# wushan270/mit-6.824-2015

Measured on AMD Instinct MI355X. Metric: word-count input GB/s (whole node) and % of HBM roofline at 1/2/4/8 MI355X, higher is better.
Workload: dtype u8

## Files before the change

__graft_entry__.py:

```python
from __future__ import annotations

import os
import shutil
import subprocess
import sys

ROOT = os.path.dirname(os.path.abspath(__file__))
PKG = os.path.join(ROOT, "mit-6.824-2015_amd")
CSRC = os.path.join(PKG, "csrc")
OUT = os.path.join(PKG, "wcg")
ORACLE = os.path.join(ROOT, "oracle")

HIPCC = os.environ.get("HIPCC", "/opt/rocm/bin/hipcc" if os.path.exists("/opt/rocm/bin/hipcc") else "hipcc")
HIP_FLAGS = ["--offload-arch=gfx950", "-O3", "-std=c++17", "-shared", "-fPIC", "-fvisibility=hidden", "-pthread"]
HIP_LIBS = ["-L/opt/rocm/lib", "-lrccl"]


def _run(cmd):
    print("+", " ".join(cmd), flush=True)
    subprocess.run(cmd, check=True)


def _stale(target, sources):
    if not os.path.exists(target):
# ... 4 lines not shown

def _sources(d, exts):
    return [os.path.join(d, f) for f in sorted(os.listdir(d)) if f.endswith(exts)]


def _check_isa() -> None:
    import tempfile
    sys.path.insert(0, os.path.join(ROOT, "tools"))
    import check_inflight
    with tempfile.TemporaryDirectory() as td:
        s = os.path.join(td, "wcg.s")
        _run([HIPCC, "--offload-arch=gfx950", "-O3", "-std=c++17", "--cuda-device-only", "-S", "-o", s,
              os.path.join(CSRC, "wcg_api.hip")])
        text = open(s).read()
    errors = []
    for sym in ("_ZN3wcg5k_mapILi0ELb1EEEvNS_7MapArgsE", "_ZN3wcg5k_mapILi0ELb0EEEvNS_7MapArgsE", "_ZN3wcg5k_aggILi0EEEvNS_7AggArgsENS_7MapArgsE",
                "_ZN3wcg5k_aggILi1EEEvNS_7AggArgsENS_7MapArgsE"):
        errors += check_inflight.check(text, sym)[0]
    if errors:
        lib = os.path.join(OUT, "libwcg.so")
        os.remove(lib)
        raise RuntimeError("k_map prefetch register discipline broken:\n" + "\n".join(errors))


def build(force: bool = False) -> None:
    hip_deps = _sources(CSRC, (".hip", ".h")) + [os.path.join(ROOT, "include", "wcg.h")]
    lib = os.path.join(OUT, "libwcg.so")
    if force or _stale(lib, hip_deps):
        _run([HIPCC, *HIP_FLAGS, "-o", lib, os.path.join(CSRC, "wcg_api.hip"), *HIP_LIBS])
        _check_isa()
    gen = os.path.join(OUT, "libgencorpus.so")
    gsrc = os.path.join(CSRC, "gencorpus.c")
# ... 45 lines not shown
```

include/wcg.h:

```cpp
#ifndef WCG_H
#define WCG_H

#include <stdint.h>

#ifdef __cplusplus
extern "C" {
#endif

#ifndef WCG_API
#define WCG_API __attribute__((visibility("default")))
#endif

typedef struct wcg_ctx wcg_ctx;

enum {
    WCG_OK = 0,
    WCG_EINVAL = 1,
    WCG_ENOMEM = 2,
    WCG_EHIP = 3,
    WCG_EFULL = 4,
    WCG_ESTATE = 5
};

enum {
// ... 81 lines not shown

WCG_API int wcg_index_merged(wcg_ctx *ctx, uint64_t *nlines);

WCG_API int wcg_load_merged(wcg_ctx *ctx, const uint8_t *host_bytes, uint64_t n, uint64_t *nlines);
WCG_API int wcg_load_merged_device(wcg_ctx *ctx, const void *dev_bytes, uint64_t n, uint64_t *nlines);

WCG_API int wcg_timings(wcg_ctx *ctx, double *ms, int n, uint64_t *map_launches);
WCG_API int wcg_enable_timing(wcg_ctx *ctx, int on);

WCG_API int wcg_stats(wcg_ctx *ctx, uint64_t *stats9);

WCG_API int wcg_ingest_stats(wcg_ctx *ctx, double *out, int n);

WCG_API int wcg_reduce_path(const wcg_ctx *ctx, int *path);

WCG_API uint32_t wcg_ihash(const uint8_t *key, uint64_t len);

WCG_API const char *wcg_version(void);

#ifdef __cplusplus
}
#endif
#endif
```

mit-6.824-2015_amd/csrc/wcg_api.hip:

```cpp
#include <hip/hip_ext.h>
#include <hip/hip_runtime.h>
#include <rccl/rccl.h>

#include <fcntl.h>
#include <sys/stat.h>
#include <unistd.h>

#include <algorithm>
#include <array>
#include <chrono>
#include <cstdio>
#include <cstdlib>
#include <cstring>
#include <memory>
#include <string>
#include <thread>
#include <tuple>
#include <vector>

#include "../../include/wcg.h"
#include "wcg_common.h"
#include "wcg_map.h"
#include "wcg_agg.h"
#include "wcg_reduce.h"
#include "wcg_top.h"
#include "wcg_query.h"
#include "wcg_index.h"
#include "wcg_fused.h"
#include "wcg_ingest.h"

using namespace wcg;

struct wcg_ctx {
    int device = 0;
    int ncu = 256;
    hipStream_t own_stream = nullptr;
    hipStream_t stream = nullptr;
    hipStream_t long_stream = nullptr;
    hipEvent_t ev_fork = nullptr, ev_join = nullptr;
    u64 max_input = 0, max_keys = 0;
    GEntry* gtab = nullptr; u64 gslots = 0;
    GEntry* ltab = nullptr; u64 lslots = 0;
    uint8_t* arena = nullptr; u64 arena_cap = 0;
// ... 102 lines not shown
    hipEvent_t phase_ev[6] = {};
    u64 map_launches_since_reset = 0;
    int timing_mode = 0;
    std::vector<std::array<hipEvent_t, 5>> phase_jobs;
    bool phase_rec = false;
    std::vector<std::tuple<int, hipEvent_t, hipEvent_t>> xev;
    double acc[10] = {};
    u64 map_launches = 0;
    uint8_t* fr_buf = nullptr;
    FrArgs fr{};
    u32 fr_epoch = 0;
    bool fused_last = false;
    bool pending = false;
    uint16_t* flist = nullptr; u64 flist_cap = 0;
    u64* h_st_dev = nullptr;
    std::string err;
};

namespace {

#define HIPCHK(ctx, call)                                                                   \
    do {                                                                                    \
        hipError_t e_ = (call);                                                             \
        if (e_ != hipSuccess) {                                                             \
            (ctx)->err = std::string(#call) + ": " + hipGetErrorString(e_);                 \
            return WCG_EHIP;                                                                \
        }                                                                                   \
    } while (0)

#define RC(call)                                                                            \
// ... 162 lines not shown
        k_compact<<<(unsigned)cdiv(std::max<u64>(total, 1), CP_NT * CP_IPT), CP_NT, 0, c->stream>>>(
            c->gtab, gs, c->ltab, ls, c->arena, c->recA, c->rec_cap, c->st, nullptr, glist, llist);
        HIPCHK(c, hipGetLastError());
        if (c->timing_all) { c->phase_ev[1] = take_event(c); HIPCHK(c, hipEventRecord(c->phase_ev[1], c->stream)); }
        RC(check_status(c));
        c->nrec = c->h_st->nrec;
        if (c->nrec <= c->rec_cap) break;
        RC(ensure_recs(c, c->nrec));
    }
    c->crec = c->recA;
    c->compacted = true;
    return WCG_OK;
}

u64 merged_bound(wcg_ctx* c, u64 n, bool json);

bool fused_eligible(wcg_ctx* c) {
    static const char* env = getenv("WCG_FUSED");
    static const bool exact_env = getenv("WCG_EXACT_REDUCE") != nullptr || getenv("WCG_SORT_TARGET") != nullptr;
    if (env && atoi(env) == 0) return false;
    return !c->compacted && !c->two_pass_used && !exact_env && c->nrec_hint >= 2 &&
           c->nrec_hint <= FR_NMAX;
}

int reduce_fused(wcg_ctx* c) {
    const u64 total = c->gslots + c->lslots;
    RC(ensure_recs(c, total));
    c->dev_sized = true;
    RC(ensure(c, &c->d_out, &c->out_cap, merged_bound(c, total, false) + 64));
    if (!c->fr_buf) {
// ... 15 lines not shown
    }
    if (!c->counts_clean) HIPCHK(c, hipMemsetAsync(&c->st->nrec, 0, 2 * sizeof(u64), c->stream));
    c->counts_clean = false;
    FrArgs a = c->fr;
    a.gtab = c->gtab; a.gslots = c->gslots; a.ltab = c->ltab; a.lslots = c->lslots;
    a.arena = c->arena; a.st = c->st; a.total_out = c->d_scalar;
    a.rec = c->recA; a.rec_cap = c->rec_cap; a.out_rec = c->recB; a.out = c->d_out;
    c->fr_epoch = (c->fr_epoch + 1) & 0xFFFFFF;
    if (c->fr_epoch == 0) c->fr_epoch = 1;
    a.epoch = c->fr_epoch;
    const char* tenv = getenv("WCG_FUSED_TARGET");
    a.target = tenv ? (u32)std::max(1, atoi(tenv)) : FR_TARGET;
    a.nitems0 = (u32)cdiv(total, (u64)CP_NT * CP_IPT);
    if (c->timing_all) { c->phase_ev[2] = take_event(c); HIPCHK(c, hipEventRecord(c->phase_ev[2], c->stream)); }
    static const bool fclock = getenv("WCG_FUSED_CLOCK") != nullptr;
    static u64* d_fclk = nullptr;
    const unsigned fgrid = (unsigned)(2 * c->ncu);
    a.clk = nullptr;
    if (fclock) {
        if (!d_fclk) HIPCHK(c, hipMalloc(&d_fclk, ((u64)fgrid * FR_CLK + 8ull * FR_NPH * FR_CLK_ITEMS + 8ull * FR_NPH) * sizeof(u64)));
        HIPCHK(c, hipMemsetAsync(d_fclk, 0, ((u64)fgrid * FR_CLK + 8ull * FR_NPH * FR_CLK_ITEMS + 8ull * FR_NPH) * sizeof(u64), c->stream));
        a.clk = d_fclk;
    }
    if (!c->h_st_dev) HIPCHK(c, hipHostGetDevicePointer((void**)&c->h_st_dev, c->h_st, 0));
    a.host_st = c->h_st_dev;
    k_fused_reduce<<<fgrid, FR_NT, 0, c->stream>>>(a);
    HIPCHK(c, hipGetLastError());
    if (fclock) {
        std::vector<u64> h((u64)fgrid * FR_CLK + 8ull * FR_NPH * FR_CLK_ITEMS + 8ull * FR_NPH);
        HIPCHK(c, hipMemcpyAsync(h.data(), d_fclk, h.size() * sizeof(u64), hipMemcpyDeviceToHost, c->stream));
        HIPCHK(c, hipStreamSynchronize(c->stream));
        u64 t0 = ~0ull, tend = 0;
        for (unsigned w = 0; w < fgrid; w++) { t0 = std::min(t0, h[w * FR_CLK]); }
        fprintf(stderr, "wcg fused clock (us from the first workgroup's start):");
        for (int p = 0; p < FR_NPH; p++) {
// ... 65 lines not shown
                std::vector<double> v = d[k];
                std::sort(v.begin(), v.end());
                fprintf(stderr, "%s %.1f/%.1f/%.1f  ", nm[k], v[v.size() / 2], v[v.size() * 9 / 10], v.back());
            }
            fprintf(stderr, "\n");
            if (!slow.empty()) {
                std::sort(slow.begin(), slow.end());
                fprintf(stderr, "  P%d slowest items (us, records):", p);
                for (size_t k = slow.size() > 6 ? slow.size() - 6 : 0; k < slow.size(); k++)
                    fprintf(stderr, " %.1f/%llu", slow[k].first, (unsigned long long)slow[k].second);
                fprintf(stderr, "; median item %.1f/%llu\n", slow[slow.size() / 2].first, (unsigned long long)slow[slow.size() / 2].second);
            }
        }
    }
    if (c->timing_all) { c->phase_ev[3] = take_event(c); HIPCHK(c, hipEventRecord(c->phase_ev[3], c->stream)); }
    c->dev_sized = false;
    c->compacted = false;
    c->fused_last = true;
    return WCG_OK;
}

int reduce_fused_finish(wcg_ctx* c) {
    HIPCHK(c, hipStreamSynchronize(c->stream));
    c->sorted = c->recB;
    c->crec = c->recA;
    c->nrec = c->nkeys = c->h_st->nrec;
    c->out_len = *c->h_scalar;
    if (c->h_st->bad_input || c->h_st->overflow || c->h_st->spin_fail) {
        c->nrec = 0; c->out_len = 0; c->reduced = false;
        RC(check_status(c));
    }
    c->nrec_hint = c->nrec;
    c->long_hint = c->h_st->long_tokens;
    c->sorted_live = true;
    c->sorted_n = c->nrec;
    return WCG_OK;
}

int resolve(wcg_ctx* c) {
    if (!c->pending) return WCG_OK;
    c->pending = false;
    return reduce_fused_finish(c);
}

int dbg(wcg_ctx* c, const char* what) {
    static const bool on = getenv("WCG_DEBUG") != nullptr;
    if (!on) return WCG_OK;
    HIPCHK(c, hipStreamSynchronize(c->stream));
    fprintf(stderr, "wcg: %s done\n", what);
    return WCG_OK;
}
// ... 469 lines not shown
    if (c->ev_fork) (void)hipEventDestroy(c->ev_fork);
    if (c->ev_join) (void)hipEventDestroy(c->ev_join);
    for (auto e : c->ev_pool) (void)hipEventDestroy(e);
    for (int i = 0; i < INGEST_SLOTS; i++) {
        if (c->ev_copied[i]) (void)hipEventDestroy(c->ev_copied[i]);
    for (auto e : c->ing_ev) (void)hipEventDestroy(e);
        if (c->ev_mapped[i]) (void)hipEventDestroy(c->ev_mapped[i]);
        if (c->hb[i]) (void)hipHostFree(c->hb[i]);
        if (c->db[i]) (void)hipFree(c->db[i]);
    }
    void* bufs[] = {c->gtab, c->ltab, c->arena, c->st, c->recA, c->recB, c->lens, c->d_out,
                    c->d_part, c->owner, c->d_per_rank, c->exp_buf, c->pool, c->region_len, c->wg_stats,
                    c->llog, c->llog_len, c->smp, c->bid, c->spx, c->irec, c->lent, c->lpcur, c->spill, c->spill_len, c->pool2, c->rlen2, c->remit, c->ovf, c->hist, c->spart, c->ikey, c->iidx, c->groups,
                    c->pid, c->d_partb, c->nlpos, c->d_rb, c->d_b0, c->d_jin, c->d_jout, c->jhist, c->dbig,
                    c->d_xrow, c->xrecv, c->grecv, c->glist, c->llist, c->fr_buf, c->flist,
                    c->top_cand, c->top_rec, c->d_top, c->q_keys, c->q_off, c->q_cnt, c->rs_part, c->d_range};
    if (c->comm) (void)ncclCommDestroy(c->comm);
    for (void* b : bufs) if (b) (void)hipFree(b);
    if (c->h_x) (void)hipHostFree(c->h_x);
    if (c->h_st) (void)hipHostFree(c->h_st);
    if (c->h_cur) (void)hipHostFree(c->h_cur);
    if (c->h_rb) (void)hipHostFree(c->h_rb);
    if (c->copy_stream) (void)hipStreamDestroy(c->copy_stream);
    if (c->own_stream) (void)hipStreamDestroy(c->own_stream);
    if (c->long_stream) (void)hipStreamDestroy(c->long_stream);
    delete c;
    return WCG_OK;
}

int wcg_set_stream(wcg_ctx* c, void* stream) {
    if (!c) return WCG_EINVAL;
// ... 161 lines not shown
            fprintf(stderr, "wcg k_agg clock: %s workgroups %u, dur mean %.1f max %.1f us, units mean %.0f\n",
                    kind ? "medium" : "short", kn[kind], kd[kind] / kn[kind] / 100.0, km[kind] / 100.0, ku[kind] / kn[kind]);
    fprintf(stderr, "wcg k_agg clock: span %.1f us, wg dur mean %.1f max %.1f us (bi %u: %llu units, start +%.1f us), "
            "units mean %.0f max %.0f\n", (t1 - t0) / 100.0, sd / nb1 / 100.0, md / 100.0, bmax,
            (unsigned long long)units[bmax], (clk[2 * bmax] - t0) / 100.0, su / nb1, mu);
    return WCG_OK;
}

}

extern "C" {

int wcg_reset(wcg_ctx* c) {
    if (!c) return WCG_EINVAL;
    c->pending = false;
    int rc = set_dev(c);
    if (rc) return rc;
    if (c->timing_mode >= 2 && c->ev_used >= EV_FOLD) {
        HIPCHK(c, hipStreamSynchronize(c->stream));
        sum_events(c, c->acc);
        c->map_ev.clear(); c->agg_ev.clear(); c->phase_jobs.clear(); c->xev.clear();
        c->ev_used = 0;
    }
    RC(reset_tables(c));
    if (c->timing_mode < 2) {
        c->map_ev.clear();
        c->agg_ev.clear();
        c->xev.clear();
        c->ev_used = 0;
        c->phase_rec = false;
// ... 79 lines not shown
        c->llog_len = nullptr; c->llog_len_cap = 0;
        HIPCHK(c, hipMalloc(&c->llog_len, grid * sizeof(u32)));
        c->llog_len_cap = grid;
    }
    a.llog = c->llog;
    a.llog_len = c->llog_len;
    const bool two_pass = two_pass0;
    const u64 rec_cap_emit = emit_log_cap(c);
    RC(ensure(c, &c->remit, &c->remit_cap, emit_log_alloc(c)));
    a.emit = two_pass ? c->remit : nullptr;
    a.emit_cap = rec_cap_emit;
    a.pool = c->pool;
    a.region_len = c->region_len;
    a.wg_stats = c->wg_stats;
    a.stamps = nullptr;
#if WCG_STAMPS
    static u64* d_stamps = nullptr;
    if (!d_stamps) HIPCHK(c, hipMalloc(&d_stamps, MAP_NSTAMP * sizeof(u64)));
    HIPCHK(c, hipMemsetAsync(d_stamps, 0, MAP_NSTAMP * sizeof(u64), c->stream));
    a.stamps = d_stamps;
#endif
    hipEvent_t e0 = nullptr, e1 = nullptr, e2 = nullptr;
    if (c->timing) { e0 = take_event(c); e1 = take_event(c); }
    static const int ablate = getenv("WCG_MAP_ABLATE") ? atoi(getenv("WCG_MAP_ABLATE")) : 0;
    auto launch = [&](auto kern) {
        if (e0) hipExtLaunchKernelGGL(kern, dim3((unsigned)grid), dim3(MAP_NT), 0, c->stream, e0, e1, 0u, a);
        else kern<<<(unsigned)grid, MAP_NT, 0, c->stream>>>(a);
    };
    switch (ablate) {
        case 1: split ? launch(k_map<1, true>) : launch(k_map<1, false>); break;
        case 2: split ? launch(k_map<2, true>) : launch(k_map<2, false>); break;
        case 3: split ? launch(k_map<3, true>) : launch(k_map<3, false>); break;
        case 4: split ? launch(k_map<4, true>) : launch(k_map<4, false>); break;
        case 5: split ? launch(k_map<5, true>) : launch(k_map<5, false>); break;
        case 6: split ? launch(k_map<6, true>) : launch(k_map<6, false>); break;
        case 7: split ? launch(k_map<7, true>) : launch(k_map<7, false>); break;
        default: split ? launch(k_map<0, true>) : launch(k_map<0, false>); break;
    }
    HIPCHK(c, hipGetLastError());
#if WCG_STAMPS
    {
        u64 h[MAP_NSTAMP];
        HIPCHK(c, hipMemcpyAsync(h, d_stamps, sizeof h, hipMemcpyDeviceToHost, c->stream));
        HIPCHK(c, hipStreamSynchronize(c->stream));
        const double ns = h[6] ? (double)h[6] : 1.0;
        fprintf(stderr, "wcg stamps (s_memtime ticks per wave step, %llu steps): loop %.0f wait %.0f mask %.0f "
                "list %.0f short %.0f general %.0f\n", (unsigned long long)h[6], h[0] / ns, h[1] / ns, h[2] / ns,
                h[3] / ns, h[4] / ns, h[5] / ns);
    }
#endif
    const bool long_path = ablate == 0 || ablate >= 6;
    static const char* fork_env = getenv("WCG_LONG_FORK");
// ... 52 lines not shown
    g.gtab = c->gtab; g.gmask = c->gslots - 1; g.st = c->st;
    g.map_stats = c->wg_stats;
    const u32 nb1 = g.nbi;
    g.spill_cap = 0;
    g.spill = nullptr; g.spill_len = nullptr;
    g.emit = c->remit; g.emit_cap = rec_cap_emit;
    g.ovf = nullptr; g.ovf_cap = 0;
    g.clk = nullptr;
    g.flist = nullptr;
    static const char* fl_env = getenv("WCG_AGG_FLIST");
    if (!two_pass && !(fl_env && atoi(fl_env) == 0)) {
        RC(ensure(c, &c->flist, &c->flist_cap, (u64)nb1 * AGG_NB * AGG_W));
        g.flist = c->flist;
    }
    static const bool agg_clock = getenv("WCG_AGG_CLOCK") != nullptr;
    static u64* d_clk = nullptr;
    if (agg_clock && !two_pass) {
        if (!d_clk) HIPCHK(c, hipMalloc(&d_clk, 2 * 65536 * sizeof(u64)));
        g.clk = nb1 <= 65536 ? d_clk : nullptr;
    }
    if (!two_pass) {
        k_agg<AGG_SPILL><<<nb1 + (small ? 1 : 0), AGG_NT, 0, c->stream>>>(g, a);
        HIPCHK(c, hipGetLastError());
        c->counts_clean = true;
        if (g.clk) RC(agg_clock_report(c, g, nb1, grid));
    } else {
    c->two_pass_used = true;
    static const char* rps_env = getenv("WCG_RP_SLICES");
    const u32 sl = std::max<u32>(1, std::min<u32>((u32)grid, rps_env ? (u32)atoi(rps_env) : 2 * g.slices));
    const u32 nrp = P * sl;
    const u64 slice_cap = (u64)cdiv(grid, sl) * a.region_cap;
// ... 141 lines not shown
    }();
    if (rc) {
        if (c->dev_sized) { c->dev_sized = false; c->compacted = false; c->nrec = 0; c->out_len = 0; }
        return rc;
    }
    if (c->dev_sized) {
        c->dev_sized = false;
        c->nrec = c->nkeys = c->h_st->nrec;
        if (c->h_st->bad_input || c->h_st->overflow || c->h_st->spin_fail) {
            c->compacted = false;
            RC(check_status(c));
        }
    }
    c->nrec_hint = c->nrec;
    if (c->h_st) c->long_hint = c->h_st->long_tokens;
    if (c->timing_all) {
        c->phase_ev[4] = take_event(c);
        HIPCHK(c, hipEventRecord(c->phase_ev[4], c->stream));
        c->phase_rec = true;
        if (c->timing_mode == 2)
            c->phase_jobs.push_back({c->phase_ev[0], c->phase_ev[1], c->phase_ev[2], c->phase_ev[3], c->phase_ev[4]});
    }
    if (c->nkeys_on_device) {
        if (c->nrec == 0) c->nkeys = 0;
        else c->nkeys = c->h_scalar[8];
        c->nkeys_on_device = false;
    }
    c->sorted_live = true;
    c->sorted_n = c->nrec;
    c->reduced = true;
// ... 980 lines not shown
            v[4] = ev_ms(c->phase_ev[3], c->phase_ev[4]);
        }
        for (auto& x : c->xev) v[std::get<0>(x)] += ev_ms(std::get<1>(x), std::get<2>(x));
    }
    for (int i = 0; i < n && i < 10; i++) ms[i] = v[i];
    if (map_launches) *map_launches = c->map_launches;
    return WCG_OK;
}

int wcg_reduce_path(const wcg_ctx* c, int* path) {
    if (!c || !path) return WCG_EINVAL;
    *path = c->fused_last ? 1 : 0;
    return WCG_OK;
}

int wcg_stats(wcg_ctx* c, uint64_t* s8) {
    if (!c || !s8) return WCG_EINVAL;
    RC(resolve(c));
    int rc = set_dev(c);
    if (rc) return rc;
    HIPCHK(c, hipMemcpyAsync(c->h_st, c->st, sizeof(DevState), hipMemcpyDeviceToHost, c->stream));
    HIPCHK(c, hipStreamSynchronize(c->stream));
    s8[0] = c->h_st->tokens; s8[1] = c->reduced ? c->nkeys : c->nrec; s8[2] = c->h_st->lds_hits; s8[3] = c->h_st->global_ops;
    s8[4] = c->h_st->long_tokens; s8[5] = c->h_st->arena_top; s8[6] = c->h_st->overflow; s8[7] = c->h_st->spin_fail;
    s8[8] = c->h_st->nemit;
    return WCG_OK;
}

}
```

mit-6.824-2015_amd/csrc/wcg_lds_table.h:

```cpp
#pragma once
#include "wcg_common.h"
#ifndef WCG_DIAG_SLOTS
#define WCG_DIAG_SLOTS 0
#endif
#ifndef WCG_MAP_ROW2
#define WCG_MAP_ROW2 0
#endif
#ifndef WCG_DIAG_NOCOUNT
#define WCG_DIAG_NOCOUNT 0
#endif

namespace wcg {

template <int NB, typename CNT, int W>
struct LdsTable {
    static_assert(W == 2 || W == 4, "rows of one or two 16-byte reads");
    u64 (*k0)[W];
    u64 (*k1)[W];
    CNT (*cnt)[W];

    struct Probe {
        u32 b1, b2;
        u64 v[W], w[W];
        u64 v1[W], w1[W];
// ... 124 lines not shown
struct MapTable {
    u64* sk0;
    u32* scnt;
    u64* mk0;
    u64* mk1;
    u32* mcnt;
    u64* zero;
    u32* seen;

    __device__ __forceinline__ void init(int tid, int nt) {
        for (int i = tid; i < NS; i += nt) { sk0[i] = 0; scnt[i] = 0; }
        for (int i = tid; i < NM; i += nt) { mk0[i] = 0; mk1[i] = 0; mcnt[i] = 0; }
        if (seen) for (int i = tid; i < (int)(ADMIT_BITS / 32); i += nt) seen[i] = 0;
        if (tid == 0) *zero = 0;
    }
    static constexpr u32 ADMIT_BITS = 16384;
    __device__ __forceinline__ bool admit(u32 h) {
        if (!seen) return true;
        const u32 b = (h * 0x9E3779B1u) >> 18;
        const u32 bit = 1u << (b & 31);
        return (atomicOr(&seen[b >> 5], bit) & bit) != 0;
    }
    __device__ __forceinline__ static void slots(u32 h, u32 n, u32& s1, u32& s2) {
#if WCG_DIAG_SLOTS
        s1 = __lane_id(); s2 = __lane_id() + 64; (void)h; (void)n;
#else
        s1 = (u32)(((u64)(h >> 8) * (u64)(n << 8)) >> 32);
        s2 = (u32)(((u64)(h & 0xFFFFFFu) * (u64)(n << 8)) >> 32);
#endif
    }
// ... 107 lines not shown
```

mit-6.824-2015_amd/csrc/wcg_map.h:

```cpp
#pragma once
#include <type_traits>

#include "wcg_common.h"
#include "wcg_lds_table.h"

namespace wcg {

#ifndef WCG_MAP_NT
#define WCG_MAP_NT 1024
#endif
#ifndef WCG_MAP_WGS
#define WCG_MAP_WGS 1
#endif
constexpr int MAP_NT = WCG_MAP_NT;
constexpr int MAP_WGS = WCG_MAP_WGS;
constexpr int MAP_WAVES = MAP_NT / 64;
constexpr int MAP_OWN = 62;
constexpr int MAP_STEP = 16 * MAP_OWN;
constexpr int MAP_WIN = 1024;
constexpr int MAP_WREG = MAP_WIN + 8;
constexpr int MAP_SST = 512;
#ifndef WCG_DIRECT
#define WCG_DIRECT 0
#endif
// ... 36 lines not shown
    u64 ntiles;
    u64 tiles_per_wg;
    GEntry* gtab;  u64 gmask;
    GEntry* ltab;  u64 lmask;
    uint8_t* arena; u64 arena_cap;
    u64 lheap_cap;
    DevState* st;
    u64* pool;     u64 region_cap;
    u32* region_len;
    u32 pmask;
    u64* wg_stats;
    u64* llog;     u32 llog_cap;
    u32* llog_len;
    Rec* emit;     u64 emit_cap;
    u64* stamps;
};
constexpr u64 LLOG_OFF_MASK = (1ull << 40) - 1;
constexpr u32 LLOG_PER_STEP = 64;

__device__ __forceinline__ bool log_push(const MapArgs& a, u32* cursor, u32 p, u64 k0, u64 k1, u32 c) {
    const u32 nu = (u32)entry_units(k0, c);
    const u32 pos = atomicAdd(&cursor[p], nu);
    u64* r = a.pool + ((u64)blockIdx.x * (a.pmask + 1) + p) * a.region_cap + pos;
    if (pos + nu <= a.region_cap) {
        put_entry(r, k0, k1, c);
        return true;
    }
    for (u32 k = pos; k < a.region_cap; k++) r[k - pos] = 0;
    return false;
}
// ... 660 lines not shown
    asm volatile("buffer_store_dwordx2 %0, %1, %2, 0 offen ; wcg-store" :: "v"(v), "v"(off), "s"(rsrc) : "memory");
}
constexpr u32 OOB = 0xFFFFFFF0u;

__device__ __forceinline__ u32 wave_incl_scan(u32 x) {
    u32 s = x + (u32)__builtin_amdgcn_update_dpp(0, (int)x, 0x111, 0xF, 0xF, true)
              + (u32)__builtin_amdgcn_update_dpp(0, (int)x, 0x112, 0xF, 0xF, true)
              + (u32)__builtin_amdgcn_update_dpp(0, (int)x, 0x113, 0xF, 0xF, true);
    s += (u32)__builtin_amdgcn_update_dpp(0, (int)s, 0x114, 0xF, 0xE, true);
    s += (u32)__builtin_amdgcn_update_dpp(0, (int)s, 0x118, 0xF, 0xC, true);
    s += (u32)__builtin_amdgcn_update_dpp(0, (int)s, 0x142, 0xA, 0xF, false);
    s += (u32)__builtin_amdgcn_update_dpp(0, (int)s, 0x143, 0xC, 0xF, false);
    return s;
}

#ifndef WCG_UTF8_LIST
#define WCG_UTF8_LIST 1
#endif
#ifndef WCG_UL_K
#define WCG_UL_K 1
#endif
#ifndef WCG_UL_MASKED
#define WCG_UL_MASKED 0
#endif
#ifndef WCG_UL_PIPE
#define WCG_UL_PIPE 1
#endif
static_assert(!WCG_UL_PIPE || WCG_UL_K == 1, "the pipelined decode rounds take one lead per lane");
constexpr int UL_K = WCG_UL_K;
__device__ __forceinline__ u32 utf8_mask_list(uint4 c, u32 nx, LdsLetters lt, const uint8_t* bytes, uint16_t* list,
// ... 150 lines not shown
    __shared__ __align__(16) u64 sk0[MAP_NS];
    __shared__ __align__(16) u64 mk0[MAP_NM];
    __shared__ __align__(16) u64 mk1[MAP_NM];
    __shared__ u64 zero_w;
    __shared__ u32 seen_w[WCG_ADMIT2 ? MapTable<MAP_NS, MAP_NM>::ADMIT_BITS / 32 : 1];
    __shared__ u32 scnt[MAP_NS];
    __shared__ u32 mcnt[MAP_NM];
    __shared__ u32 cursor[MAX_MISS_BUCKETS];
    __shared__ u32 lcur;
    __shared__ uint8_t lt_idx[LT_LDS_BLOCKS + 4];
    __shared__ u32 lt_bits[WCG_LT_NBLOCKS * 8];

    const int tid = threadIdx.x, lane = tid & 63;
    const int wave = __builtin_amdgcn_readfirstlane(tid >> 6);
    MapTable<MAP_NS, MAP_NM> tab{sk0, scnt, mk0, mk1, mcnt, &zero_w, WCG_ADMIT2 ? seen_w : nullptr};
    tab.init(tid, MAP_NT);
    for (int i = tid; i < MAX_MISS_BUCKETS; i += MAP_NT) cursor[i] = 0;
    if (tid == 0) lcur = 0;
    lds_letters_init(lt_idx, lt_bits, tid, MAP_NT);
    __syncthreads();
    const LdsLetters lt{lt_idx, lt_bits};

#if !WCG_DIRECT
    uint8_t* const bytes = wbytes[wave];
    uint16_t* const sst = wstart[wave];
#endif
    u64 stp[MAP_NSTAMP] = {};
    u64 t_last = WCG_STAMPS ? __builtin_amdgcn_s_memtime() : 0;
    auto stamp = [&](int i) {
        if (WCG_STAMPS) { const u64 t = __builtin_amdgcn_s_memtime(); stp[i] += t - t_last; t_last = t; }
    };
// ... 505 lines not shown
```

mit-6.824-2015_amd/wcg/_lib.py:

```python
from __future__ import annotations

import ctypes
import os
from typing import List, Optional, Sequence, Tuple

_HERE = os.path.dirname(os.path.abspath(__file__))
LIB_PATH = os.environ.get("WCG_LIB") or os.path.join(_HERE, "libwcg.so")

WCG_OK, WCG_EINVAL, WCG_ENOMEM, WCG_EHIP, WCG_EFULL, WCG_ESTATE = range(6)
RECORD_BYTES = 32

_lib: Optional[ctypes.CDLL] = None

EXPORTED = [
    "wcg_open", "wcg_close", "wcg_last_error", "wcg_set_stream", "wcg_reset", "wcg_map",
    "wcg_map_device", "wcg_reduce", "wcg_result_device", "wcg_result_copy", "wcg_partition",
    "wcg_export", "wcg_import", "wcg_timings", "wcg_enable_timing", "wcg_stats", "wcg_ihash",
    "wcg_version", "wcg_map_file", "wcg_partition_all", "wcg_map_json", "wcg_export_count",
    "wcg_export_write", "wcg_merge_runs", "wcg_result_copy_device", "wcg_sync", "wcg_free",
    "wcg_comm_id", "wcg_comm_init", "wcg_exchange", "wcg_gather_merge", "wcg_exchange_plan",
    "wcg_gather_plan", "wcg_exchange_local", "wcg_gather_merge_local", "wcg_reduce_path",
    "wcg_reduce_async", "wcg_reduce_wait", "wcg_ingest_stats", "wcg_top", "wcg_map_size_check",
    "wcg_lookup", "wcg_lookup_device", "wcg_range", "wcg_index_merged", "wcg_load_merged",
    "wcg_load_merged_device",
]
COMM_ID_BYTES = 128
TOP_MAX = 1024


class WcgError(RuntimeError):

    def __init__(self, status: int, msg: str):
        super().__init__(f"wcg status {status}: {msg}")
        self.status = status


def load() -> ctypes.CDLL:
    global _lib
    if _lib is not None:
# ... 39 lines not shown
        "wcg_gather_plan": (I, [PU64, U32, U32, PU64, PU64]),
        "wcg_exchange_local": (I, [ctypes.POINTER(P), U32, U32, PU64, PU64]),
        "wcg_gather_merge_local": (I, [ctypes.POINTER(P), U32, U32, PU64, PU64]),
        "wcg_reduce_path": (I, [P, ctypes.POINTER(I)]),
        "wcg_reduce_async": (I, [P]),
        "wcg_reduce_wait": (I, [P, PU64, PU64]),
        "wcg_ingest_stats": (I, [P, ctypes.POINTER(ctypes.c_double), I]),
        "wcg_top": (I, [P, U32, P, U64, PU64, PU64]),
        "wcg_map_size_check": (I, [U64]),
        "wcg_lookup": (I, [P, ctypes.c_char_p, PU64, U64, PU64]),
        "wcg_lookup_device": (I, [P, P, P, U64, P]),
        "wcg_range": (I, [P, ctypes.c_char_p, U64, ctypes.c_char_p, U64, P, U64, PU64, PU64]),
        "wcg_index_merged": (I, [P, PU64]),
        "wcg_load_merged": (I, [P, ctypes.c_char_p, U64, PU64]),
        "wcg_load_merged_device": (I, [P, P, U64, PU64]),
    }
    for name, (res, args) in sig.items():
        fn = getattr(lib, name)
        fn.restype = res
        fn.argtypes = args
    _lib = lib
    return lib


_hiprt = None


def _hip() -> ctypes.CDLL:
    global _hiprt
    if _hiprt is None:
        for name in ("libamdhip64.so", "/opt/rocm/lib/libamdhip64.so"):
            try:
# ... 278 lines not shown
        self._chk(self._lib.wcg_timings(self._ctx, ms, 10, ctypes.byref(nl)))
        return dict(zip(self.PHASES, list(ms))), nl.value

    def reduce_path(self) -> int:
        v = ctypes.c_int()
        self._chk(self._lib.wcg_reduce_path(self._ctx, ctypes.byref(v)))
        return v.value

    INGEST_STATS = ["host_issue_ms", "read_ms", "slot_wait_ms", "copy_ms", "copy_span_ms",
                    "copy_engine_idle_frac", "map_ms", "device_span_ms", "chunks"]

    def ingest_stats(self) -> dict:
        v = (ctypes.c_double * len(self.INGEST_STATS))()
        self._chk(self._lib.wcg_ingest_stats(self._ctx, v, len(self.INGEST_STATS)))
        return dict(zip(self.INGEST_STATS, list(v)))

    def stats(self) -> dict:
        s = (ctypes.c_uint64 * 9)()
        self._chk(self._lib.wcg_stats(self._ctx, s))
        keys = ["tokens", "keys", "lds_hits", "global_ops", "long_tokens", "arena_bytes", "overflow",
                "spin_fail", "emitted"]
        return dict(zip(keys, list(s)))


def _slices(raw: bytes, sizes: List[int]) -> List[bytes]:
    out, off = [], 0
    for n in sizes:
        out.append(raw[off:off + n])
        off += n
    return out
# ... 140 lines not shown
```

Baseline: 1155.

## Seed per-block LDS hash tables with hot keys from the previous job

After a job reduces, three new kernels histogram record counts, pick the most frequent short and medium keys, and place them into a table image in device memory. Later map launches copy that image into each block's LDS table instead of starting empty, with counts zeroed, so frequent words hit in LDS rather than falling through to global atomics. The image is rebuilt when the LDS hit rate drops below the rate recorded at build time. This adds build kernels and one host sync on the first seeded job, and helps only when later jobs share a vocabulary with earlier ones.

```diff
diff --git a/__graft_entry__.py b/__graft_entry__.py
--- a/__graft_entry__.py
+++ b/__graft_entry__.py
@@ -42,8 +42,8 @@
               os.path.join(CSRC, "wcg_api.hip")])
         text = open(s).read()
     errors = []
-    for sym in ("_ZN3wcg5k_mapILi0ELb1EEEvNS_7MapArgsE", "_ZN3wcg5k_mapILi0ELb0EEEvNS_7MapArgsE", "_ZN3wcg5k_aggILi0EEEvNS_7AggArgsENS_7MapArgsE",
-                "_ZN3wcg5k_aggILi1EEEvNS_7AggArgsENS_7MapArgsE"):
+    for sym in ("_ZN3wcg5k_mapILi0ELb1EEEvNS_7MapArgsE", "_ZN3wcg5k_mapILi0ELb0EEEvNS_7MapArgsE", "_ZN3wcg5k_mapILi8ELb1EEEvNS_7MapArgsE",
+                "_ZN3wcg5k_aggILi0EEEvNS_7AggArgsENS_7MapArgsE", "_ZN3wcg5k_aggILi1EEEvNS_7AggArgsENS_7MapArgsE"):
         errors += check_inflight.check(text, sym)[0]
     if errors:
         lib = os.path.join(OUT, "libwcg.so")
diff --git a/include/wcg.h b/include/wcg.h
--- a/include/wcg.h
+++ b/include/wcg.h
@@ -119,6 +119,8 @@
 
 WCG_API int wcg_reduce_path(const wcg_ctx *ctx, int *path);
 
+WCG_API int wcg_seed_stats(wcg_ctx *ctx, uint64_t *stats3);
+
 WCG_API uint32_t wcg_ihash(const uint8_t *key, uint64_t len);
 
 WCG_API const char *wcg_version(void);
diff --git a/mit-6.824-2015_amd/csrc/wcg_api.hip b/mit-6.824-2015_amd/csrc/wcg_api.hip
--- a/mit-6.824-2015_amd/csrc/wcg_api.hip
+++ b/mit-6.824-2015_amd/csrc/wcg_api.hip
@@ -27,6 +27,7 @@
 #include "wcg_query.h"
 #include "wcg_index.h"
 #include "wcg_fused.h"
+#include "wcg_seed.h"
 #include "wcg_ingest.h"
 
 using namespace wcg;
@@ -159,6 +160,15 @@
     bool pending = false;
     uint16_t* flist = nullptr; u64 flist_cap = 0;
     u64* h_st_dev = nullptr;
+    u64* seed = nullptr;
+    bool seed_ok = false;
+    double seed_rate = -1.0;
+    bool job_seeded = false, job_unseeded = false, job_built = false;
+    bool last_seeded = false;
+    u64 seed_builds = 0;
+    u64* d_clk = nullptr;
+    u64* d_fclk = nullptr;
+    u64* d_stamps = nullptr;
     std::string err;
 };
 
@@ -351,6 +361,51 @@
 }
 
 u64 merged_bound(wcg_ctx* c, u64 n, bool json);
+
+bool seed_on(const wcg_ctx* c) {
+    const char* e = getenv("WCG_SEED");
+    return !(e && atoi(e) == 0) && !c->two_pass_used && !c->imported;
+}
+
+int seed_build(wcg_ctx* c, const Rec* rec, u64 ncap, const u64* dev_n, u64 nhint) {
+    if (!c->seed) HIPCHK(c, hipMalloc(&c->seed, SEED_ALLOC_BYTES));
+    SeedScratch* sc = reinterpret_cast<SeedScratch*>(c->seed + SEED_IMG_WORDS);
+    HIPCHK(c, hipMemsetAsync(sc, 0, SEED_ZERO_BYTES, c->stream));
+    const int grid = grid_for(std::max<u64>(nhint, 1), SEED_NT, 2 * c->ncu);
+    k_seed_hist<<<grid, SEED_NT, 0, c->stream>>>(rec, ncap, dev_n, sc);
+    k_seed_pick<<<grid, SEED_NT, 0, c->stream>>>(rec, ncap, dev_n, sc);
+    k_seed_place<<<1, SEED_PLACE_NT, 0, c->stream>>>(sc, c->seed, c->st);
+    HIPCHK(c, hipGetLastError());
+    c->seed_ok = true;
+    c->seed_builds++;
+    if (getenv("WCG_DEBUG")) fprintf(stderr, "wcg seed: build %llu\n", (unsigned long long)c->seed_builds);
+    return WCG_OK;
+}
+
+bool seed_wanted(const wcg_ctx* c) { return seed_on(c) && !c->seed_ok && c->job_unseeded; }
+
+int seed_job_done(wcg_ctx* c) {
+    const bool built = c->job_built;
+    c->job_built = false;
+    c->last_seeded = c->job_seeded && !c->job_unseeded;
+    if (!c->seed_ok) return WCG_OK;
+    const u64 tokens = c->h_st->tokens;
+    const double rate = tokens ? (double)c->h_st->lds_hits / (double)tokens : -1.0;
+    if (built) { c->seed_rate = rate; return WCG_OK; }
+    if (!c->last_seeded || rate < 0) return WCG_OK;
+    if (c->seed_rate < 0) {
+        u64 job[2] = {0, 0};
+        const SeedScratch* sc = reinterpret_cast<const SeedScratch*>(c->seed + SEED_IMG_WORDS);
+        HIPCHK(c, hipMemcpyAsync(job, sc->job, sizeof job, hipMemcpyDeviceToHost, c->stream));
+        HIPCHK(c, hipStreamSynchronize(c->stream));
+        c->seed_rate = job[0] ? (double)job[1] / (double)job[0] : 0.0;
+    }
+    if (rate < c->seed_rate) {
+        c->seed_ok = false;
+        if (getenv("WCG_DEBUG")) fprintf(stderr, "wcg seed: stale (%.4f < %.4f), dropped\n", rate, c->seed_rate);
+    }
+    return WCG_OK;
+}
 
 bool fused_eligible(wcg_ctx* c) {
     static const char* env = getenv("WCG_FUSED");
@@ -396,11 +451,11 @@
     a.nitems0 = (u32)cdiv(total, (u64)CP_NT * CP_IPT);
     if (c->timing_all) { c->phase_ev[2] = take_event(c); HIPCHK(c, hipEventRecord(c->phase_ev[2], c->stream)); }
     static const bool fclock = getenv("WCG_FUSED_CLOCK") != nullptr;
-    static u64* d_fclk = nullptr;
+    u64*& d_fclk = c->d_fclk;
     const unsigned fgrid = (unsigned)(2 * c->ncu);
     a.clk = nullptr;
     if (fclock) {
-        if (!d_fclk) HIPCHK(c, hipMalloc(&d_fclk, ((u64)fgrid * FR_CLK + 8ull * FR_NPH * FR_CLK_ITEMS + 8ull * FR_NPH) * sizeof(u64)));
+        if (!d_fclk) HIPCHK(c, hipMalloc(&d_fclk,((u64)fgrid * FR_CLK + 8ull * FR_NPH * FR_CLK_ITEMS + 8ull * FR_NPH) * sizeof(u64)));
         HIPCHK(c, hipMemsetAsync(d_fclk, 0, ((u64)fgrid * FR_CLK + 8ull * FR_NPH * FR_CLK_ITEMS + 8ull * FR_NPH) * sizeof(u64), c->stream));
         a.clk = d_fclk;
     }
@@ -496,6 +551,10 @@
         }
     }
     if (c->timing_all) { c->phase_ev[3] = take_event(c); HIPCHK(c, hipEventRecord(c->phase_ev[3], c->stream)); }
+    if (seed_wanted(c)) {
+        RC(seed_build(c, c->recB, c->rec_cap, &c->st->nrec, c->nrec_hint));
+        c->job_built = true;
+    }
     c->dev_sized = false;
     c->compacted = false;
     c->fused_last = true;
@@ -510,13 +569,14 @@
     c->out_len = *c->h_scalar;
     if (c->h_st->bad_input || c->h_st->overflow || c->h_st->spin_fail) {
         c->nrec = 0; c->out_len = 0; c->reduced = false;
+        if (c->job_built) { c->job_built = false; c->seed_ok = false; }
         RC(check_status(c));
     }
     c->nrec_hint = c->nrec;
     c->long_hint = c->h_st->long_tokens;
     c->sorted_live = true;
     c->sorted_n = c->nrec;
-    return WCG_OK;
+    return seed_job_done(c);
 }
 
 int resolve(wcg_ctx* c) {
@@ -1016,7 +1076,8 @@
                     c->llog, c->llog_len, c->smp, c->bid, c->spx, c->irec, c->lent, c->lpcur, c->spill, c->spill_len, c->pool2, c->rlen2, c->remit, c->ovf, c->hist, c->spart, c->ikey, c->iidx, c->groups,
                     c->pid, c->d_partb, c->nlpos, c->d_rb, c->d_b0, c->d_jin, c->d_jout, c->jhist, c->dbig,
                     c->d_xrow, c->xrecv, c->grecv, c->glist, c->llist, c->fr_buf, c->flist,
-                    c->top_cand, c->top_rec, c->d_top, c->q_keys, c->q_off, c->q_cnt, c->rs_part, c->d_range};
+                    c->top_cand, c->top_rec, c->d_top, c->q_keys, c->q_off, c->q_cnt, c->rs_part, c->d_range,
+                    c->seed, c->d_clk, c->d_fclk, c->d_stamps};
     if (c->comm) (void)ncclCommDestroy(c->comm);
     for (void* b : bufs) if (b) (void)hipFree(b);
     if (c->h_x) (void)hipHostFree(c->h_x);
@@ -1208,6 +1269,7 @@
 int wcg_reset(wcg_ctx* c) {
     if (!c) return WCG_EINVAL;
     c->pending = false;
+    c->job_seeded = c->job_unseeded = c->job_built = false;
     int rc = set_dev(c);
     if (rc) return rc;
     if (c->timing_mode >= 2 && c->ev_used >= EV_FOLD) {
@@ -1317,15 +1379,18 @@
     a.region_len = c->region_len;
     a.wg_stats = c->wg_stats;
     a.stamps = nullptr;
+    static const int ablate = getenv("WCG_MAP_ABLATE") ? atoi(getenv("WCG_MAP_ABLATE")) : 0;
+    const bool seeded = split && ablate == 0 && c->seed_ok && seed_on(c);
+    a.seed = seeded ? c->seed : nullptr;
+    (seeded ? c->job_seeded : c->job_unseeded) = true;
 #if WCG_STAMPS
-    static u64* d_stamps = nullptr;
+    u64*& d_stamps = c->d_stamps;
     if (!d_stamps) HIPCHK(c, hipMalloc(&d_stamps, MAP_NSTAMP * sizeof(u64)));
     HIPCHK(c, hipMemsetAsync(d_stamps, 0, MAP_NSTAMP * sizeof(u64), c->stream));
     a.stamps = d_stamps;
 #endif
     hipEvent_t e0 = nullptr, e1 = nullptr, e2 = nullptr;
     if (c->timing) { e0 = take_event(c); e1 = take_event(c); }
-    static const int ablate = getenv("WCG_MAP_ABLATE") ? atoi(getenv("WCG_MAP_ABLATE")) : 0;
     auto launch = [&](auto kern) {
         if (e0) hipExtLaunchKernelGGL(kern, dim3((unsigned)grid), dim3(MAP_NT), 0, c->stream, e0, e1, 0u, a);
         else kern<<<(unsigned)grid, MAP_NT, 0, c->stream>>>(a);
@@ -1338,7 +1403,10 @@
         case 5: split ? launch(k_map<5, true>) : launch(k_map<5, false>); break;
         case 6: split ? launch(k_map<6, true>) : launch(k_map<6, false>); break;
         case 7: split ? launch(k_map<7, true>) : launch(k_map<7, false>); break;
-        default: split ? launch(k_map<0, true>) : launch(k_map<0, false>); break;
+        default:
+            if (seeded) launch(k_map<MAP_SEEDED, true>);
+            else split ? launch(k_map<0, true>) : launch(k_map<0, false>);
+            break;
     }
     HIPCHK(c, hipGetLastError());
 #if WCG_STAMPS
@@ -1421,7 +1489,7 @@
         g.flist = c->flist;
     }
     static const bool agg_clock = getenv("WCG_AGG_CLOCK") != nullptr;
-    static u64* d_clk = nullptr;
+    u64*& d_clk = c->d_clk;
     if (agg_clock && !two_pass) {
         if (!d_clk) HIPCHK(c, hipMalloc(&d_clk, 2 * 65536 * sizeof(u64)));
         g.clk = nb1 <= 65536 ? d_clk : nullptr;
@@ -1593,6 +1661,11 @@
     }
     c->nrec_hint = c->nrec;
     if (c->h_st) c->long_hint = c->h_st->long_tokens;
+    if (c->nrec && seed_wanted(c)) {
+        RC(seed_build(c, c->sorted, c->nrec, nullptr, c->nrec));
+        c->job_built = true;
+    }
+    RC(seed_job_done(c));
     if (c->timing_all) {
         c->phase_ev[4] = take_event(c);
         HIPCHK(c, hipEventRecord(c->phase_ev[4], c->stream));
@@ -2603,6 +2676,15 @@
     return WCG_OK;
 }
 
+int wcg_seed_stats(wcg_ctx* c, uint64_t* s3) {
+    if (!c || !s3) return WCG_EINVAL;
+    RC(resolve(c));
+    s3[0] = c->seed_ok ? 1 : 0;
+    s3[1] = c->seed_builds;
+    s3[2] = c->last_seeded ? 1 : 0;
+    return WCG_OK;
+}
+
 int wcg_stats(wcg_ctx* c, uint64_t* s8) {
     if (!c || !s8) return WCG_EINVAL;
     RC(resolve(c));
diff --git a/mit-6.824-2015_amd/csrc/wcg_lds_table.h b/mit-6.824-2015_amd/csrc/wcg_lds_table.h
--- a/mit-6.824-2015_amd/csrc/wcg_lds_table.h
+++ b/mit-6.824-2015_amd/csrc/wcg_lds_table.h
@@ -162,6 +162,19 @@
         if (seen) for (int i = tid; i < (int)(ADMIT_BITS / 32); i += nt) seen[i] = 0;
         if (tid == 0) *zero = 0;
     }
+    __device__ __forceinline__ void init_seeded(const u64* img, int tid, int nt) {
+        static_assert(NS % 2 == 0 && NM % 2 == 0, "16-byte copies");
+        const uint4* s = reinterpret_cast<const uint4*>(img);
+        for (int i = tid; i < NS / 2; i += nt) reinterpret_cast<uint4*>(sk0)[i] = s[i];
+        for (int i = tid; i < NM / 2; i += nt) {
+            reinterpret_cast<uint4*>(mk0)[i] = s[NS / 2 + i];
+            reinterpret_cast<uint4*>(mk1)[i] = s[NS / 2 + NM / 2 + i];
+        }
+        for (int i = tid; i < NS; i += nt) scnt[i] = 0;
+        for (int i = tid; i < NM; i += nt) mcnt[i] = 0;
+        if (seen) for (int i = tid; i < (int)(ADMIT_BITS / 32); i += nt) seen[i] = 0;
+        if (tid == 0) *zero = 0;
+    }
     static constexpr u32 ADMIT_BITS = 16384;
     __device__ __forceinline__ bool admit(u32 h) {
         if (!seen) return true;
diff --git a/mit-6.824-2015_amd/csrc/wcg_map.h b/mit-6.824-2015_amd/csrc/wcg_map.h
--- a/mit-6.824-2015_amd/csrc/wcg_map.h
+++ b/mit-6.824-2015_amd/csrc/wcg_map.h
@@ -74,6 +74,7 @@
     u32* llog_len;
     Rec* emit;     u64 emit_cap;
     u64* stamps;
+    const u64* seed;
 };
 constexpr u64 LLOG_OFF_MASK = (1ull << 40) - 1;
 constexpr u32 LLOG_PER_STEP = 64;
@@ -764,6 +765,7 @@
     return s;
 }
 
+constexpr int MAP_SEEDED = 8;
 #ifndef WCG_UTF8_LIST
 #define WCG_UTF8_LIST 1
 #endif
@@ -944,7 +946,8 @@
     const int tid = threadIdx.x, lane = tid & 63;
     const int wave = __builtin_amdgcn_readfirstlane(tid >> 6);
     MapTable<MAP_NS, MAP_NM> tab{sk0, scnt, mk0, mk1, mcnt, &zero_w, WCG_ADMIT2 ? seen_w : nullptr};
-    tab.init(tid, MAP_NT);
+    if (ABL == MAP_SEEDED) tab.init_seeded(a.seed, tid, MAP_NT);
+    else tab.init(tid, MAP_NT);
     for (int i = tid; i < MAX_MISS_BUCKETS; i += MAP_NT) cursor[i] = 0;
     if (tid == 0) lcur = 0;
     lds_letters_init(lt_idx, lt_bits, tid, MAP_NT);
diff --git a/mit-6.824-2015_amd/csrc/wcg_seed.h b/mit-6.824-2015_amd/csrc/wcg_seed.h
--- /dev/null
+++ b/mit-6.824-2015_amd/csrc/wcg_seed.h
@@ -0,0 +1,170 @@
+#pragma once
+#include "wcg_common.h"
+#include "wcg_lds_table.h"
+#include "wcg_map.h"
+
+namespace wcg {
+
+constexpr u32 SEED_NUM = 3, SEED_DEN = 4;
+constexpr u32 SEED_TS = (u32)MAP_NS * SEED_NUM / SEED_DEN;
+constexpr u32 SEED_TM = (u32)MAP_NM * SEED_NUM / SEED_DEN;
+constexpr u32 SEED_NCAND = SEED_TS + SEED_TM;
+constexpr u32 SEED_BINS = 64;
+constexpr u64 SEED_IMG_WORDS = (u64)MAP_NS + 2ull * MAP_NM;
+static_assert(MAP_NS % 2 == 0 && MAP_NM % 2 == 0, "the image is copied 16 bytes at a time");
+
+struct SeedScratch {
+    u32 hist[2][SEED_BINS];
+    u32 ctr[2][2];
+    u64 job[2];
+    u32 bin[SEED_NCAND];
+    u64 k0[SEED_NCAND];
+    u64 k1[SEED_NCAND];
+};
+constexpr u64 SEED_ZERO_BYTES = sizeof(u32) * (2 * SEED_BINS + 4);
+constexpr u64 SEED_ALLOC_BYTES = SEED_IMG_WORDS * sizeof(u64) + sizeof(SeedScratch);
+
+constexpr int SEED_NT = 256;
+constexpr int SEED_PLACE_NT = 1024;
+constexpr u32 SEED_CPT = (SEED_NCAND + SEED_PLACE_NT - 1) / SEED_PLACE_NT;
+
+__device__ __forceinline__ u64 seed_nrec(u64 ncap, const u64* dev_n) {
+    if (!dev_n) return ncap;
+    const u64 n = *dev_n;
+    return n < ncap ? n : ncap;
+}
+
+__device__ __forceinline__ bool seed_kind_bin(u64 cnt, u64 ref, u32& kind, u32& bin) {
+    if (ref == 0 || ref > 15 || cnt == 0) return false;
+    kind = ref >= 8 ? 1u : 0u;
+    bin = 63u - (u32)__builtin_clzll(cnt);
+    return true;
+}
+
+__device__ __forceinline__ void seed_threshold(const u32* hist, u32 target, u32& T, u32& above, u32& take) {
+    u32 acc = 0;
+    for (int b = SEED_BINS - 1; b >= 0; b--) {
+        const u32 hb = hist[b];
+        if (acc + hb >= target || b == 0) {
+            T = (u32)b;
+            above = acc;
+            take = hb < target - acc ? hb : target - acc;
+            return;
+        }
+        acc += hb;
+    }
+}
+
+__device__ __forceinline__ u32 seed_reserve(u32* ctr, bool want) {
+    const u64 m = __ballot(want);
+    if (m == 0) return 0;
+    const u32 rank = __builtin_amdgcn_mbcnt_hi((u32)(m >> 32), __builtin_amdgcn_mbcnt_lo((u32)m, 0u));
+    const int leader = __builtin_ctzll(m);
+    u32 base = 0;
+    if ((int)(threadIdx.x & 63) == leader) base = atomicAdd(ctr, (u32)__popcll(m));
+    return (u32)__shfl((int)base, leader, 64) + rank;
+}
+
+__global__ __launch_bounds__(SEED_NT) void k_seed_hist(const Rec* rec, u64 ncap, const u64* dev_n, SeedScratch* sc) {
+    __shared__ u32 lh[2 * SEED_BINS];
+    for (int i = threadIdx.x; i < 2 * (int)SEED_BINS; i += SEED_NT) lh[i] = 0;
+    __syncthreads();
+    const u64 n = seed_nrec(ncap, dev_n);
+    for (u64 i = (u64)blockIdx.x * SEED_NT + threadIdx.x; i < n; i += (u64)gridDim.x * SEED_NT) {
+        const ulonglong2 cr = *reinterpret_cast<const ulonglong2*>(&rec[i].cnt);
+        u32 kind, bin;
+        if (seed_kind_bin(cr.x, cr.y, kind, bin)) atomicAdd(&lh[kind * SEED_BINS + bin], 1u);
+    }
+    __syncthreads();
+    for (int i = threadIdx.x; i < 2 * (int)SEED_BINS; i += SEED_NT)
+        if (lh[i]) atomicAdd(&sc->hist[0][0] + i, lh[i]);
+}
+
+__global__ __launch_bounds__(SEED_NT) void k_seed_pick(const Rec* rec, u64 ncap, const u64* dev_n, SeedScratch* sc) {
+    __shared__ u32 sT[2], sAbove[2], sTake[2];
+    if (threadIdx.x < 2)
+        seed_threshold(sc->hist[threadIdx.x], threadIdx.x ? SEED_TM : SEED_TS, sT[threadIdx.x], sAbove[threadIdx.x],
+                       sTake[threadIdx.x]);
+    __syncthreads();
+    const u64 n = seed_nrec(ncap, dev_n);
+    for (u64 base = (u64)blockIdx.x * SEED_NT; base < n; base += (u64)gridDim.x * SEED_NT) {
+        const u64 i = base + threadIdx.x;
+        Rec r{0, 0, 0, 0};
+        if (i < n) r = rec[i];
+        u32 kind = 0, bin = 0;
+        const bool ok = seed_kind_bin(r.cnt, r.ref, kind, bin);
+#pragma unroll
+        for (u32 kd = 0; kd < 2; kd++) {
+            const bool mine = ok && kind == kd;
+            const bool hi = mine && bin > sT[kd], at = mine && bin == sT[kd];
+            const u32 ph = seed_reserve(&sc->ctr[kd][0], hi);
+            const u32 pa = seed_reserve(&sc->ctr[kd][1], at);
+            const u32 target = kd ? SEED_TM : SEED_TS;
+            u32 pos = target;
+            if (hi) pos = ph;
+            if (at && pa < sTake[kd]) pos = sAbove[kd] + pa;
+            if (pos < target) {
+                const u32 q = (kd ? SEED_TS : 0u) + pos;
+                u64 k0, k1;
+                rec_inline_key(r, k0, k1);
+                sc->k0[q] = k0; sc->k1[q] = k1; sc->bin[q] = bin;
+            }
+        }
+    }
+}
+
+__global__ __launch_bounds__(SEED_PLACE_NT) void k_seed_place(SeedScratch* sc, u64* img, const DevState* st) {
+    __shared__ __align__(16) u64 sk0[MAP_NS];
+    __shared__ __align__(16) u64 mk0[MAP_NM];
+    __shared__ __align__(16) u64 mk1[MAP_NM];
+    __shared__ u32 sN[2], sLo, sHi;
+    const int tid = threadIdx.x;
+    for (int i = tid; i < MAP_NS; i += SEED_PLACE_NT) sk0[i] = 0;
+    for (int i = tid; i < MAP_NM; i += SEED_PLACE_NT) { mk0[i] = 0; mk1[i] = 0; }
+    if (tid < 2) {
+        u32 T, above, take;
+        seed_threshold(sc->hist[tid], tid ? SEED_TM : SEED_TS, T, above, take);
+        sN[tid] = above + take;
+    }
+    if (tid == 0) {
+        sc->job[0] = st->tokens;
+        sc->job[1] = st->lds_hits;
+        u32 lo = SEED_BINS, hi = 0;
+        for (u32 b = 0; b < SEED_BINS; b++)
+            if (sc->hist[0][b] | sc->hist[1][b]) { if (lo == SEED_BINS) lo = b; hi = b; }
+        sLo = lo; sHi = hi;
+    }
+    __syncthreads();
+    u64 k0[SEED_CPT], k1[SEED_CPT];
+    u32 bin[SEED_CPT];
+#pragma unroll
+    for (u32 j = 0; j < SEED_CPT; j++) {
+        const u32 q = j * SEED_PLACE_NT + tid;
+        const bool live = q < SEED_TS ? q < sN[0] : (q < SEED_NCAND && q - SEED_TS < sN[1]);
+        k0[j] = live ? sc->k0[q] : 0;
+        k1[j] = live ? sc->k1[q] : 0;
+        bin[j] = live ? sc->bin[q] : SEED_BINS;
+    }
+    using Tab = MapTable<MAP_NS, MAP_NM>;
+    if (sLo < SEED_BINS)
+    for (int b = (int)sHi; b >= (int)sLo; b--) {
+#pragma unroll
+        for (u32 j = 0; j < SEED_CPT; j++) {
+            if (bin[j] != (u32)b) continue;
+            const bool med = !key_short(k0[j]);
+            const u32 h = lds_hash(k0[j], k1[j]);
+            u32 s1, s2;
+            Tab::slots(h, med ? (u32)MAP_NM : (u32)MAP_NS, s1, s2);
+            u64* const K0 = med ? mk0 : sk0;
+            u32 s = s1;
+            u64 old = atomicCAS(&K0[s], 0ull, k0[j]);
+            if (old != 0) { s = s2; old = atomicCAS(&K0[s], 0ull, k0[j]); }
+            if (old == 0 && med) mk1[s] = k1[j];
+        }
+        __syncthreads();
+    }
+    for (int i = tid; i < MAP_NS; i += SEED_PLACE_NT) img[i] = sk0[i];
+    for (int i = tid; i < MAP_NM; i += SEED_PLACE_NT) { img[MAP_NS + i] = mk0[i]; img[MAP_NS + MAP_NM + i] = mk1[i]; }
+}
+
+}
diff --git a/mit-6.824-2015_amd/wcg/_lib.py b/mit-6.824-2015_amd/wcg/_lib.py
--- a/mit-6.824-2015_amd/wcg/_lib.py
+++ b/mit-6.824-2015_amd/wcg/_lib.py
@@ -22,7 +22,7 @@
     "wcg_gather_plan", "wcg_exchange_local", "wcg_gather_merge_local", "wcg_reduce_path",
     "wcg_reduce_async", "wcg_reduce_wait", "wcg_ingest_stats", "wcg_top", "wcg_map_size_check",
     "wcg_lookup", "wcg_lookup_device", "wcg_range", "wcg_index_merged", "wcg_load_merged",
-    "wcg_load_merged_device",
+    "wcg_load_merged_device", "wcg_seed_stats",
 ]
 COMM_ID_BYTES = 128
 TOP_MAX = 1024
@@ -92,8 +92,11 @@
         "wcg_index_merged": (I, [P, PU64]),
         "wcg_load_merged": (I, [P, ctypes.c_char_p, U64, PU64]),
         "wcg_load_merged_device": (I, [P, P, U64, PU64]),
+        "wcg_seed_stats": (I, [P, PU64]),
     }
     for name, (res, args) in sig.items():
+        if os.environ.get("WCG_LIB") and not hasattr(lib, name):
+            continue
         fn = getattr(lib, name)
         fn.restype = res
         fn.argtypes = args
@@ -402,6 +405,11 @@
         v = (ctypes.c_double * len(self.INGEST_STATS))()
         self._chk(self._lib.wcg_ingest_stats(self._ctx, v, len(self.INGEST_STATS)))
         return dict(zip(self.INGEST_STATS, list(v)))
+
+    def seed_stats(self) -> dict:
+        s = (ctypes.c_uint64 * 3)()
+        self._chk(self._lib.wcg_seed_stats(self._ctx, s))
+        return {"valid": bool(s[0]), "builds": int(s[1]), "last_job_seeded": bool(s[2])}
 
     def stats(self) -> dict:
         s = (ctypes.c_uint64 * 9)()
```

Result: faster. 1171 (median of 6 runs) (+1.4%).
